# littlepure2333/GFlow

Measured on AMD Instinct MI355X. Metric: GFlow fit_video frames/sec (fwd+bwd+step) @60k Gaussians 480p, higher is better.
Workload: dtype f32

## Files before the change

gflow_amd/_lib.py:

```python
import ctypes
import os
import subprocess
import threading

import torch

_HERE = os.path.dirname(os.path.abspath(__file__))
_CSRC = os.path.join(_HERE, "csrc")
LIB_PATH = os.environ.get("GFLOW_HIP_LIB") or os.path.join(_HERE, "libgflow_hip.so")

_lock = threading.Lock()
_lib = None

c_void_p, c_int, c_float, c_size_t, c_int64 = ctypes.c_void_p, ctypes.c_int, ctypes.c_float, ctypes.c_size_t, ctypes.c_int64

MIN_VERSION = 312

_P = c_void_p
SIGNATURES = {
    "gfl_version": (c_int, []),
    "gfl_constants": (c_int, [_P]),
    "gfl_constants_n": (c_int, [_P, c_int]),
    "gfl_ewa_on_mfma": (c_int, []),
    "gfl_status_string": (ctypes.c_char_p, [c_int]),
# ... 26 lines not shown
    "gfl_step_increment": (c_int, [_P, _P]),
    "gfl_tile_sort_only": (c_int, [_P, c_int, c_int, _P, _P, _P, _P]),
    "gfl_tile_sort_ordered": (c_int, [_P, c_int, c_int, c_int, _P, _P, _P, _P]),
    "gfl_tile_sort_reserved": (c_int, [_P, _P, _P, _P, c_int, c_int, c_int, _P, _P, _P, _P]),
    "gfl_fit_workspace_bytes": (c_size_t, [c_int, c_int, c_int, c_int]),
    "gfl_fit_workspace_layout": (c_int, [c_int, c_int, c_int, c_int, _P, _P, _P, c_int]),
    "gfl_fit_forward": (c_int, [_P, _P, _P]),
    "gfl_fit_backward_step": (c_int, [_P, _P, _P]),
    "gfl_fit_iteration": (c_int, [_P, _P, _P]),
    "gfl_fit_iterations": (c_int, [_P, _P, c_int, c_int, _P]),
    "gfl_fit_reserved_supported": (c_int, [_P, _P]),
    "gfl_fit_snapshot_stage": (c_int, [_P, _P, _P]),
    "gfl_fit_snapshot_workspace_bytes": (c_size_t, [c_int, c_int, c_int]),
    "gfl_fit_snapshot": (c_int, [_P, _P, _P, _P, _P, c_size_t, _P]),
    "gfl_fit_iteration_snapshot": (c_int, [_P, _P, _P, _P, _P]),
    "gfl_render_fwd": (c_int, [_P, _P, _P]),
    "gfl_render_bwd": (c_int, [_P, _P, _P, _P, _P, _P, _P, _P]),
    "gfl_render_bwd_cam": (c_int, [_P, _P, _P, _P, _P, _P, _P, _P, _P]),
    "gfl_render_batch_workspace_bytes": (c_size_t, [c_int, c_int, c_int, c_int, c_int]),
    "gfl_render_batch": (c_int, [_P, c_int, _P, _P, c_int, c_int, c_int, c_int, c_int, _P, _P, _P, _P, _P, c_size_t, _P]),
    "gfl_fit_prepare_targets": (c_int, [_P, _P]),
    "gfl_fit_schedule_info": (c_int, [_P, _P, _P, _P, _P]),
    "gfl_fit_schedule_info_fwd": (c_int, [_P, _P, _P, _P, _P]),
    "gfl_selftest_reduce10": (c_int, [_P, _P, _P, _P]),
    "gfl_selftest_cov2d": (c_int, [_P, _P, c_int, _P, _P, _P]),
    "gfl_selftest_block_mask": (c_int, [_P, c_int, c_int, c_int, c_int, _P, _P, _P]),
    "gfl_concave_hull": (c_int, [_P, c_int, ctypes.c_double, ctypes.c_double, _P, c_int]),
    "gfl_scan_f64_workspace_bytes": (c_size_t, [c_int]),
    "gfl_scan_f64": (c_int, [_P, c_int, _P, _P, c_size_t, _P]),
    "gfl_track_anchor_workspace_bytes": (c_size_t, [c_int, c_int]),
# ... 142 lines not shown
```

gflow_amd/csrc/gfl_fit.hip:

```cpp
#include "gfl_fit_blend.hpp"

using namespace gfl;

extern "C" {

size_t gfl_loss_workspace_bytes(int W, int H);

static inline int fit_nblk(int N) { return (N + BIN_BLOCK - 1) / BIN_BLOCK; }

static bool ewa_on_mfma() {
    static const bool on = [] { const char* e = getenv("GFL_EWA_MFMA"); return e && e[0] == '1'; }();
    return on;
}

int gfl_ewa_on_mfma(void) { return ewa_on_mfma() ? 1 : 0; }

static int fwd_split_min() {
    static const int v = [] { const char* e = getenv("GFL_FWD_SPLIT_MIN"); return e ? atoi(e) : FWD_SPLIT_MIN; }();
    return v;
}

static bool reserved_enabled() {
    static const bool on = [] { const char* e = getenv("GFL_RESERVED"); return !(e && e[0] == '0'); }();
    return on;
}

static int device_cus() {
    static const int cus = [] {
        int dev = 0, n = 0;
        const bool ok = hipGetDevice(&dev) == hipSuccess &&
                        hipDeviceGetAttribute(&n, hipDeviceAttributeMultiprocessorCount, dev) == hipSuccess && n > 0;
        return ok ? n : 256;
    }();
    return cus;
// ... 155 lines not shown
static PreArgs pre_args(const gfl_fit_state* st, const gfl_fit_hyper* hp, const FitWs& w, int gx, int gy, int op_mode) {
    PreArgs a;
    a.intr = st->intr; a.pose = st->pose;
    a.N = st->N; a.W = st->W; a.H = st->H;
    a.nearest = hp->nearest; a.extent = hp->extent;
    a.gx = gx; a.gy = gy;
    a.rec = st->rec; a.wide_off = w.wide_off; a.hist_g = w.hist; a.extr_out = st->extr; a.overflow = st->overflow;
    a.pool_counter = w.pool_counter; a.pool_cap = st->K_cap;
    a.op_mode = op_mode;
    a.scale_rows_mode = (!op_mode && hp->lambda_scale != 0.f) ? (hp->freeze_all_splats ? 2 : 1) : 0;
    a.scale_cnt = w.scale_cnt;
    return a;
}

static int fit_forward_impl(const gfl_fit_state* st, const gfl_fit_hyper* hp, gfl_stream_t stream, int op_mode, int reserved = 0,
                            const float* snap_lut = nullptr, uint8_t* snap_u8 = nullptr) {
    int rc = fit_check(st, hp);
    if (rc) return rc;
    hipStream_t s = (hipStream_t)stream;
    const auto [gx, gy, T] = tile_grid(st->W, st->H);
    const FitWs w = carve(st);
    const int nblk = fit_nblk(st->N > 0 ? st->N : 1);
    if ((size_t)T * sizeof(int32_t) > 57 * 1024) return GFL_ERR_INVALID;
    const PreArgs pa = pre_args(st, hp, w, gx, gy, op_mode);
    if (reserved) {
        if (op_mode || !fit_reserved_ok(w, T)) return GFL_ERR_INVALID;
        {
            StageScope p(ST_PREPROCESS, s);
            BinArgs b;
            b.region = w.region; b.fill = w.fill; b.keys = w.keys; b.K_cap = st->K_cap;
            b.regions_valid = w.regions_valid; b.extent_next = w.extent_next; b.extent = w.extent;
// ... 27 lines not shown
                                           stream);
            else
                rc = gfl_tile_sort_only(st->tile_offsets, gx * gy, st->K_cap, w.keys, st->ids, st->tile_range, stream);
        }
        if (rc) return rc;
    }
    {
        StageScope p(ST_BLEND_FWD, s);
        const TileQueue q = {w.sched_fwd.list, w.sched_fwd.count, w.sched.counters, w.sched.nq, w.sched.cap_q};
        if (snap_u8) {
            rc = check(hipMemsetAsync(w.snap_mm, 0, 2 * sizeof(unsigned), s));
            if (rc) return rc;
            if (st->N > 0) launch_rec_depth_range(st->rec, st->N, w.snap_mm, s);
            launch_blend_fwd(st, hp->bg, gx, blend_grid(st, T, FWD_WG_PER_CU), st->render, st->final_T, st->n_contrib, q, w, 2,
                             w.snap_mm, snap_lut, fwd_split_min(), s, snap_u8);
            launch_center_blend(st, hp->bg, gx, T, nullptr, snap_u8 + (size_t)2 * st->W * st->H * 3, s);
        }
        const bool foot = st->foot_flags && !(hp->bg > 0.f) && st->N > 0;
        if (foot && !st->keep) return GFL_ERR_INVALID;
        const bool foot_inside = foot && !snap_u8;
        if (!snap_u8)
            launch_blend_fwd(st, hp->bg, gx, blend_grid(st, T, FWD_WG_PER_CU), st->render, st->final_T, st->n_contrib, q, w,
                             foot_inside ? 3 : 0, nullptr, nullptr, fwd_split_min(), s);
        if (st->foot_flags) {
            if (!st->keep) return GFL_ERR_INVALID;
            if (foot && !foot_inside) launch_footprint(st, gx, T, s);
        }
    }
    return check_launch();
}

// ... 15 lines not shown
}

int gfl_fit_snapshot(const gfl_fit_state* st, const gfl_fit_hyper* hp, const float* lut, uint8_t* out_u8, void* workspace,
                     size_t workspace_bytes, gfl_stream_t stream) {
    int rc = fit_check(st, hp);
    if (rc) return rc;
    if (!lut || !out_u8 || !workspace) return GFL_ERR_INVALID;
    if (workspace_bytes < gfl_fit_snapshot_workspace_bytes(st->N, st->W, st->H)) return GFL_ERR_WORKSPACE;
    hipStream_t s = (hipStream_t)stream;
    const auto [gx, gy, T] = tile_grid(st->W, st->H);
    const FitWs w = carve(st);
    const SnapWs sw = snap_ws(workspace, st->W, st->H);
    rc = check(hipMemsetAsync(workspace, 0, sw.head_bytes, s));
    if (rc) return rc;
    if (st->N > 0) launch_rec_depth_range(st->rec, st->N, sw.mm, s);
    launch_center_blend(st, hp->bg, gx, T, sw.img_c, nullptr, s);
    {
        const TileQueue q = {w.sched_fwd.list, w.sched_fwd.count, sw.pull, w.sched.nq, w.sched.cap_q};
        launch_blend_fwd(st, hp->bg, gx, blend_grid(st, T, FWD_WG_PER_CU), sw.img_dc, sw.fT, sw.nc, q, w, 1, sw.mm, lut, fwd_split_min(), s);
    }
    launch_snapshot_u8(st->render, sw.img_dc, sw.img_c, st->W * st->H, out_u8, s);
    return check_launch();
}

int gfl_fit_snapshot_stage(const gfl_fit_state* src, const gfl_fit_state* dst, gfl_stream_t stream) {
    if (!src || !dst || !src->workspace || !dst->workspace || !src->rec || !dst->rec || !src->ids || !dst->ids ||
        !src->tile_range || !dst->tile_range || !src->render || !dst->render || !src->tile_offsets)
        return GFL_ERR_INVALID;
    if (src->W != dst->W || src->H != dst->H || src->N != dst->N || dst->N > dst->cap || src->N > src->cap)
        return GFL_ERR_INVALID;
    if (!fit_ws_fits(src) || !fit_ws_fits(dst)) return GFL_ERR_WORKSPACE;
// ... 4 lines not shown
    StageCopy c;
    c.k_ptr = a.extent;
    c.ids_cap = (unsigned)min(src->K_cap, dst->K_cap);
    c.seg[0] = {(const uint32_t*)src->ids, (uint32_t*)dst->ids, 0u};
    c.seg[1] = {(const uint32_t*)src->rec, (uint32_t*)dst->rec, (unsigned)((size_t)src->N * REC)};
    c.seg[2] = {(const uint32_t*)src->tile_range, (uint32_t*)dst->tile_range, (unsigned)(2 * T)};
    c.seg[3] = {(const uint32_t*)src->render, (uint32_t*)dst->render, (unsigned)(3 * P)};
    c.seg[4] = {(const uint32_t*)a.sched_fwd.list, (uint32_t*)b.sched_fwd.list,
                (unsigned)((size_t)a.sched_fwd.nq * a.sched_fwd.cap_q)};
    c.seg[5] = {(const uint32_t*)a.sched_fwd.count, (uint32_t*)b.sched_fwd.count, (unsigned)a.sched_fwd.nq};
    c.seg[6] = {(const uint32_t*)a.sched.first_slot, (uint32_t*)b.sched.first_slot, (unsigned)T};
    launch_snapshot_stage(c, (hipStream_t)stream);
    return check_launch();
}

int gfl_render_fwd(const gfl_fit_state* st, const gfl_fit_hyper* hp, gfl_stream_t stream) {
    if (st && st->foot_flags) return GFL_ERR_INVALID;
    if (st && (st->flags & GFL_FIT_DETERMINISTIC)) {
        const int rc = fit_check(st, hp);
        if (rc) return rc;
        const int T = tile_grid(st->W, st->H).T;
        const FitWs w = carve(st);
        hipStream_t s = (hipStream_t)stream;
        if (check(hipMemsetAsync(w.sched.work, 0, 4 * (size_t)T * sizeof(int32_t), s)) ||
            check(hipMemsetAsync(w.sched_fwd.work, 0, 4 * (size_t)T * sizeof(int32_t), s)) ||
            check(hipMemsetAsync(w.sched_valid, 0, sizeof(int32_t), s)))
            return GFL_ERR_HIP;
    }
    return fit_forward_impl(st, hp, stream, 1);
}
// ... 103 lines not shown
    if (rc) return rc;
    const int T = tile_grid(st->W, st->H).T;
    const FitWs w = carve(st);
    const bool res_ok = fit_reserved_ok(w, T) && st->N > 0;
    if ((flags & GFL_ITER_RESERVED) && !res_ok) return GFL_ERR_INVALID;
    for (int j = 0; j < count; ++j) {
        const int reserved = res_ok && (j > 0 || (flags & GFL_ITER_RESERVED)) ? 1 : 0;
        rc = fit_forward_impl(st, hp, stream, 0, reserved);
        if (rc) return rc;
        rc = gfl_fit_backward_step(st, hp, stream);
        if (rc) return rc;
    }
    return GFL_OK;
}

int gfl_fit_iteration_snapshot(const gfl_fit_state* st, const gfl_fit_hyper* hp, const float* lut, uint8_t* out_u8,
                               gfl_stream_t stream) {
    if (!lut || !out_u8) return GFL_ERR_INVALID;
    int rc = fit_forward_impl(st, hp, stream, 0, 0, lut, out_u8);
    if (rc) return rc;
    return gfl_fit_backward_step(st, hp, stream);
}

int gfl_fit_reserved_supported(const gfl_fit_state* st, const gfl_fit_hyper* hp) {
    if (fit_check(st, hp) || st->N <= 0) return 0;
    const int T = tile_grid(st->W, st->H).T;
    return fit_reserved_ok(carve(st), T) ? 1 : 0;
}

int gfl_fit_prepare_targets(const gfl_fit_state* st, gfl_stream_t stream) {
    if (!st || st->W <= 0 || st->H <= 0 || !st->gt_rgb || !st->workspace) return GFL_ERR_INVALID;
    if (!fit_ws_fits(st)) return GFL_ERR_WORKSPACE;
    const FitWs w = carve(st);
    return gfl_loss_prepare_gt(st->gt_rgb, st->keep, st->W, st->H, w.gt_stats, stream);
}

// ... 41 lines not shown
```

gflow_amd/csrc/gfl_fit.hpp:

```cpp
#pragma once
#include "gfl_math.hpp"
#include "gfl_profile.hpp"
#include "gfl_sched.hpp"

#include <stdlib.h>

namespace gfl {

constexpr int BIN_BLOCK = 512;
#ifndef GFL_RBIN_BLOCK
#define GFL_RBIN_BLOCK 512
#endif
constexpr int RBIN_BLOCK = GFL_RBIN_BLOCK;
static_assert(RBIN_BLOCK == 256 || RBIN_BLOCK == 512, "two scale-row partials per 512 splats (PreArgs.scale_cnt)");
#ifndef GFL_WIDE_TILES
#define GFL_WIDE_TILES 16
#endif
constexpr int WIDE_TILES = GFL_WIDE_TILES;
constexpr int ROW = 16;
constexpr int REC = 12;
#ifndef GFL_PG_STRIDE
#define GFL_PG_STRIDE 12
#endif
constexpr int PG = GFL_PG_STRIDE;
// ... 145 lines not shown
    unsigned long long* keys;
    int K_cap;
    int32_t* regions_valid;
    const int32_t* extent_next;
    int32_t* extent;
    int32_t* pull_counters; int n_pull;
};

__host__ __device__ __forceinline__ int region_cap(int c) { return c + (c >> 2) + 32; }
struct ReserveOut { int4* region; int32_t* fill; int32_t* extent_next; int32_t* total; int K_cap; };

constexpr int BLEND_WG_PER_CU = 8;
constexpr int FWD_WG_PER_CU = 5;
constexpr int FWD_UNITS = 4;
constexpr int FWD_SPLIT_MIN = 448;
constexpr int FB = 256;
#ifndef GFL_FWD_LONG_BATCH
#define GFL_FWD_LONG_BATCH 256
#endif
constexpr int FBL = GFL_FWD_LONG_BATCH;
constexpr int FBB = 192;
constexpr int FBB_DET = 64;

struct WgVote {
    int32_t* cnt;
    int base0, base1, round;
};
__device__ __forceinline__ WgVote wg_vote_init(int32_t* lds2) {
    WgVote v;
    v.cnt = lds2; v.base0 = 0; v.base1 = 0; v.round = 0;
// ... 245 lines not shown
}

struct StageSeg { const uint32_t* src; uint32_t* dst; unsigned n; };
struct StageCopy { StageSeg seg[7]; const int32_t* k_ptr; unsigned ids_cap; };

void launch_preprocess_fwd(const float* params, const PreArgs& a, const uint8_t* row_flags, int nblk, bool mfma, hipStream_t s);
void launch_preprocess_bin(const float* params, const PreArgs& a, const uint8_t* row_flags, const BinArgs& b, int nblk, bool mfma,
                           hipStream_t s);
void launch_colscan(const FitWs& w, int nblk, int T, int32_t* overflow, hipStream_t s);
void launch_scatter(const gfl_fit_state* st, const FitWs& w, int nblk, int gx, int gy, bool ordered, hipStream_t s);
inline unsigned inv_of(int gx) { return (unsigned)((((unsigned long long)1 << 32) + (unsigned)gx - 1) / (unsigned)gx); }
void launch_blend_fwd(const gfl_fit_state* st, float bg, int gx, int grid, float* out, float* final_T, int32_t* n_contrib,
                      const TileQueue& q, const FitWs& w, int mode, const unsigned* cmap_mm, const float* cmap_lut, int split_min,
                      hipStream_t s, uint8_t* snap_u8 = nullptr);
void launch_footprint(const gfl_fit_state* st, int gx, int T, hipStream_t s);
void launch_center_blend(const gfl_fit_state* st, float bg, int gx, int T, float* out, uint8_t* out_u8, hipStream_t s);
void launch_rec_depth_range(const float* rec, int N, unsigned* mm, hipStream_t s);
void launch_snapshot_u8(const float* a, const float* b, const float* c, int P, uint8_t* out, hipStream_t s);
void launch_snapshot_stage(const StageCopy& c, hipStream_t s);
void launch_blend_bwd(const gfl_fit_state* st, float bg, int gx, int gy, int grid, int sums, const float* d_out, const TileQueue& q,
                      const FitWs& w, const LossTail& lt, hipStream_t s);
void launch_splat_bwd_adam(const gfl_fit_state* st, const FitWs& w, int gx, int gy, const RegCfg& rc, const AdamCfg& ac,
                           const NextSched& ns, int extra, size_t lds, hipStream_t s);
void launch_splat_bwd_op(const gfl_fit_state* st, const FitWs& w, int gx, int gy, const NextSched& ns, int extra, size_t lds,
                         const float* d_uv, const float* d_depth, float* d_params, float* d_extr, hipStream_t s);
void launch_splat_bwd_op_cam(const gfl_fit_state* st, const FitWs& w, int gx, int gy, const NextSched& ns, int extra, size_t lds,
                             const float* d_uv, const float* d_depth, float* d_params, float* d_extr, float* d_intr, hipStream_t s);
void launch_camera_adam(const gfl_fit_state* st, const FitWs& w, int rows, const float* p_ssim, int n_ssim, const float* p_grad,
                        int n_grad, const AdamCfg& ac_cam, const AdamCfg& ac_ab, int step_camera, hipStream_t s);
#ifdef GFL_TRACE
int read_phase_trace_bin(long long* out, int n_values);
// ... 8 lines not shown
```

gflow_amd/csrc/gfl_fit_snap.hip:

```cpp
#include "gfl_fit.hpp"

namespace gfl {

__global__ void __launch_bounds__(256) center_blend_kernel(const float* __restrict__ rec, const int32_t* __restrict__ ids,
                                                           const int32_t* __restrict__ tile_range, float bg, int W, int H, int gx,
                                                           float* __restrict__ out, uint8_t* __restrict__ out_u8) {
    __shared__ RecLDS recs[FB + 1];
    __shared__ unsigned char s_mask[FB];
    const int tile = blockIdx.x;
    const int tx = tile % gx, ty = tile / gx;
    const TilePixel px = tile_pixel(tx, ty, W, H);
    const float blob_cutoff = alpha_cutoff(1.f, 1.f);
    float T, a[3];
    plain_tile_blend<3>(ids, tile_range[2 * tile], tile_range[2 * tile + 1], tx, ty, pixf(px.px), pixf(px.py), px.inside, recs, s_mask,
                        [&](int g, float4& p0, float4& p1, float4& p2) {
                            const float4* r4 = reinterpret_cast<const float4*>(rec + (size_t)g * REC);
                            p0 = r4[0]; p1 = r4[1]; p2 = r4[2];
                            p0.z = 1.f; p0.w = 0.f; p1.x = 1.f; p1.y = 1.f;
                            p2.z = p2.z < 0.f ? p2.z : blob_cutoff;
                        }, T, a);
    if (px.inside) {
        const size_t pix = (size_t)px.py * W + px.px, plane = (size_t)H * W;
        const float o0 = fmaf(T, bg, a[0]), o1 = fmaf(T, bg, a[1]), o2 = fmaf(T, bg, a[2]);
        if (out_u8) {
            uint8_t* u = out_u8 + pix * 3;
            u[0] = img_u8(o0); u[1] = img_u8(o1); u[2] = img_u8(o2);
        } else {
            out[pix] = o0; out[plane + pix] = o1; out[2 * plane + pix] = o2;
        }
    }
}

__global__ void __launch_bounds__(256) rec_depth_range_kernel(const float* __restrict__ rec, int N, unsigned* __restrict__ mm) {
    unsigned lo = 0xffffffffu, hi = 0u;
    for (int i = blockIdx.x * blockDim.x + threadIdx.x; i < N; i += gridDim.x * blockDim.x) {
        const float x = rec[(size_t)i * REC + 9];
        const unsigned b = __float_as_uint(x);
// ... 29 lines not shown
__global__ void __launch_bounds__(256) snapshot_stage_kernel(StageCopy c) {
    const unsigned tid = blockIdx.x * blockDim.x + threadIdx.x, stride = gridDim.x * blockDim.x;
#pragma unroll
    for (int sgi = 0; sgi < 7; ++sgi) {
        const StageSeg sg = c.seg[sgi];
        unsigned n = sg.n;
        if (sgi == 0) n = min((unsigned)max(*c.k_ptr, 0), c.ids_cap);
        const unsigned n4 = n >> 2;
        const uint4* s4 = reinterpret_cast<const uint4*>(sg.src);
        uint4* d4 = reinterpret_cast<uint4*>(sg.dst);
        for (unsigned i = tid; i < n4; i += stride) d4[i] = s4[i];
        for (unsigned i = (n4 << 2) + tid; i < n; i += stride) sg.dst[i] = sg.src[i];
    }
}

void launch_center_blend(const gfl_fit_state* st, float bg, int gx, int T, float* out, uint8_t* out_u8, hipStream_t s) {
    center_blend_kernel<<<T, 256, 0, s>>>(st->rec, st->ids, st->tile_range, bg, st->W, st->H, gx, out, out_u8);
}

void launch_rec_depth_range(const float* rec, int N, unsigned* mm, hipStream_t s) {
    rec_depth_range_kernel<<<min((N + 255) / 256, 32), 256, 0, s>>>(rec, N, mm);
}

void launch_snapshot_u8(const float* a, const float* b, const float* c, int P, uint8_t* out, hipStream_t s) {
    snapshot_u8_kernel<<<(P + 255) / 256, 256, 0, s>>>(a, b, c, P, out);
}

void launch_snapshot_stage(const StageCopy& c, hipStream_t s) { snapshot_stage_kernel<<<1024, 256, 0, s>>>(c); }

}
```

gflow_amd/fused.py:

```python
import ctypes

import torch

from . import _lib as L
from .pinned import DeferredRead

ROW = 16
REC = 12
COLS = {"xyz": (0, 3), "scale": (3, 6), "rotate": (6, 10), "opacity": (10, 11), "rgb": (11, 14)}

_P = ctypes.c_void_p
_I = ctypes.c_int32


class FitState(ctypes.Structure):
    _fields_ = [("N", _I), ("cap", _I), ("W", _I), ("H", _I), ("K_cap", _I), ("gt_cached", _I),
                ("params", _P), ("adam_m", _P), ("adam_v", _P), ("rec", _P), ("d_rec", _P),
                ("flow_target", _P), ("flow_w", _P), ("still_target", _P), ("still_w", _P), ("row_flags", _P),
                ("pose", _P), ("pose_m", _P), ("pose_v", _P),
                ("depth_ab", _P), ("depth_ab_m", _P), ("depth_ab_v", _P),
                ("intr", _P), ("extr", _P), ("d_extr", _P), ("step", _P),
                ("gt_rgb", _P), ("gt_depth", _P), ("keep", _P), ("move_mask", _P), ("foot_flags", _P),
                ("render", _P), ("final_T", _P), ("n_contrib", _P),
                ("d_render", _P), ("err_px", _P), ("sums", _P),
# ... 15 lines not shown
def _declare(lib):
    if getattr(lib, "_fit_declared", False):
        return
    lib.gfl_fit_workspace_bytes.restype = ctypes.c_size_t
    lib.gfl_fit_workspace_bytes.argtypes = [ctypes.c_int] * 4
    for name in ("gfl_fit_forward", "gfl_fit_backward_step", "gfl_fit_iteration", "gfl_render_fwd"):
        fn = getattr(lib, name)
        fn.restype = ctypes.c_int
        fn.argtypes = [ctypes.POINTER(FitState), ctypes.POINTER(FitHyper), _P]
    lib.gfl_fit_iterations.restype = ctypes.c_int
    lib.gfl_fit_iterations.argtypes = [ctypes.POINTER(FitState), ctypes.POINTER(FitHyper), ctypes.c_int, ctypes.c_int, _P]
    lib.gfl_fit_snapshot.restype = ctypes.c_int
    lib.gfl_fit_snapshot.argtypes = [ctypes.POINTER(FitState), ctypes.POINTER(FitHyper), _P, _P, _P, ctypes.c_size_t, _P]
    lib.gfl_fit_iteration_snapshot.restype = ctypes.c_int
    lib.gfl_fit_iteration_snapshot.argtypes = [ctypes.POINTER(FitState), ctypes.POINTER(FitHyper), _P, _P, _P]
    lib.gfl_render_bwd.restype = ctypes.c_int
    lib.gfl_render_bwd.argtypes = [ctypes.POINTER(FitState), ctypes.POINTER(FitHyper), _P, _P, _P, _P, _P, _P]
    lib.gfl_render_bwd_cam.restype = ctypes.c_int
    lib.gfl_render_bwd_cam.argtypes = [ctypes.POINTER(FitState), ctypes.POINTER(FitHyper), _P, _P, _P, _P, _P, _P, _P]
    lib._fit_declared = True


PROFILE = {"mask": 0}

import gc as _gc
import threading as _threading

_GRAPH_LOCK = _threading.RLock()


# ... 274 lines not shown
        L.check(self.lib.gfl_fit_backward_step(ctypes.byref(self.state()), ctypes.byref(self.hp), L.stream()),
                "fit backward/step")
        self._reserved_N = self.N

    GFL_ITER_RESERVED = 8

    def _reserved_flag(self):
        if self._reserved_N != self.N or self.N <= 0:
            return 0
        key = (self.W, self.H, self.K_cap)
        if self._reserved_sup[0] != key:
            self._reserved_sup = (key, int(self.lib.gfl_fit_reserved_supported(ctypes.byref(self.state()),
                                                                                ctypes.byref(self.hp))))
        return self.GFL_ITER_RESERVED if self._reserved_sup[1] else 0

    def iteration(self, use_graph=False, count=1, snapshot=False, flags=0, reserved=None):
        if snapshot:
            from .color import lut
            assert count == 1
            if self._snap_out is None:
                self._snap_out = torch.empty(3, self.H, self.W, 3, dtype=torch.uint8, device=self.dev)
            snap_args = (L.ptr(lut("turbo", self.dev)), L.ptr(self._snap_out))
        reserved = 0 if (flags or reserved is False or snapshot) else self._reserved_flag()
        st, hp = self.state(), self.hp
        fn, args, what = ((self.lib.gfl_fit_iteration_snapshot, snap_args, "snapshot iteration") if snapshot else
                          (self.lib.gfl_fit_iterations, (count, int(flags) | reserved), "fit iterations"))
        launch = lambda: L.check(fn(ctypes.byref(st), ctypes.byref(hp), *args, L.stream()), what)
        if use_graph and not PROFILE["mask"] and self._launched and not flags:
            gkey = ("snap", count, reserved) if snapshot else (count, reserved)
            g = self.graphs.lookup(bytes(st) + bytes(hp), gkey)
            if g is None:
                g = self.graphs.capture(gkey, launch)
            g.replay()
        else:
            launch()
            self._launched = True
        self._reserved_N = self.N
        return self._snap_out if snapshot else None

    def snapshot(self, out=None):
        from .color import lut
        need = self.lib.gfl_fit_snapshot_workspace_bytes(self.N, self.W, self.H)
        if self._snap_ws is None or self._snap_ws.numel() < need:
            self._snap_ws = torch.empty(int(need * 1.5), dtype=torch.uint8, device=self.dev)
        if out is None:
            out = torch.empty(3, self.H, self.W, 3, dtype=torch.uint8, device=self.dev)
        L.check(self.lib.gfl_fit_snapshot(ctypes.byref(self.state()), ctypes.byref(self.hp), L.ptr(lut("turbo", self.dev)),
                                          L.ptr(out), L.ptr(self._snap_ws), self._snap_ws.numel(), L.stream()), "snapshot")
        return out

    _STATE_TENSORS = ("step", "pose", "pose_m", "pose_v", "depth_ab", "ab_m", "ab_v")

    def save_state(self):
        n = self.N
        out = {"N": n, "rows": [t[:n].clone() for t in (self.params, self.adam_m, self.adam_v)]}
        for k in self._STATE_TENSORS:
            out[k] = getattr(self, k).clone()
        return out

    def restore_state(self, saved):
        n = saved["N"]
        if n != self.N:
            raise RuntimeError("FitEngine.restore_state: the splat count has changed since save_state")
        self._reserved_N = -1
# ... 116 lines not shown
```

gflow_amd/stage.py:

```python
from types import SimpleNamespace

import torch

from . import geometry, losses
from . import render as render_mod
from .optim import LinearLR
from .pinned import PINNED, copy_stream


class StagePlan(SimpleNamespace):

    def snapshot(self, i):
        return bool(self.snapshot_interval) and i % self.snapshot_interval == 0

    def log(self, i):
        return bool(self.log_interval) and i % self.log_interval == 0

    def occ_densify(self, i):
        return bool(self.occlusion) and i == 0

    def err_densify(self, i):
        return bool(not self.camera_only and self.densify_interval and (i + 1) % self.densify_interval == 0
                    and (i + 1) // self.densify_interval <= self.densify_times)

# ... 267 lines not shown
                last()

    def account(self):
        k = self.eng.take_pending()
        if k is None:
            if self.unchecked:
                self.settle()
        elif k < 0:
            self.settle()
        else:
            for _ in range(k):
                self.eng.iteration(use_graph=False, reserved=False)

    def _launch(self, dst, n_rendered, looked_at):
        tr, eng = self.tr, self.eng
        if dst is not None and not tr.async_snapshots:
            imgs = eng.iteration(use_graph=tr.use_graph, snapshot=True, reserved=False)
            torch.bitwise_or(imgs, 0, out=dst)
        else:
            eng.iteration(use_graph=tr.use_graph, reserved=None if not looked_at else False)
            if dst is not None:
                tr._snapshot_async(dst, n_rendered)
                self.sink.snap_stream = tr._snap_stream

    def one_iteration(self):
        tr, eng, p, iteration = self.tr, self.eng, self.plan, self.iteration
        n_rendered = eng.N
        looked_at = not p.plain(iteration)
        if looked_at and tr.exact_snapshots:
            self.account()
        if self.tentative:
            tr.rasterisations_done += 1
        dst = None
        if p.snapshot(iteration):
            dst = self.sink.slot(len(self.frames))
        launch = lambda: self._launch(dst, n_rendered, looked_at)
        launch()
        if looked_at and tr.exact_snapshots == "blocking":
# ... 73 lines not shown
```

gflow_amd/trainer.py:

```python
import math
import os

import numpy as np
import torch
import torch.nn as nn
import torch.nn.functional as F

from . import _lib as L
from . import geometry, msplat
from . import render as render_mod
from .geometry import device_constant, pose_to_extr, rotmat_to_unitquat_xyzw
from .optim import Adam
from .pinned import PINNED
from .sampling import complex_texture_sampling
from .stage import FusedStage, OperatorStage, StagePlan


def run_to_end(g):
    try:
        while True:
            next(g)
    except StopIteration as e:
        return e.value


class SimpleGaussian:
    def __init__(self, gt_image, gt_depth=None, gt_flow=None, num_points=100000, background="black",
                 device=None, log_dir=None, seed=None, fused=True, deterministic=None):
        self.fused = bool(fused)
        self.deterministic = L.resolve_deterministic(deterministic)
        if self.deterministic and not self.fused and deterministic is not None:
            raise ValueError("SimpleGaussian(deterministic=True) needs fused=True: the operator path's alpha_blending "
                             "backward has no deterministic implementation")
        self.async_snapshots = True
        self.exact_snapshots = True
        self.cu_count = 0
        self.use_graph = True
        self.engine = None
        self.device = torch.device(device if device is not None else "cuda")
        if self.device.type != "cuda":
            raise RuntimeError("gflow_amd.trainer needs a HIP device (there is no CPU rasteriser)")
        self.gt_image = gt_image.to(self.device)
        self.gt_depth = gt_depth.to(self.device) if gt_depth is not None else None
        self.gt_flow = gt_flow.to(self.device) if gt_flow is not None else None
        self.num_points = num_points
        H, W, _ = gt_image.shape
        self.H, self.W = H, W
        self.bg = {"black": 0.0, "white": 1.0, "cyan": 0.33}.get(background, 0.0)
        fov = math.pi / 2.0
# ... 267 lines not shown
        return run_to_end(self.train_steps(*a, **kw))

    def train_steps(self, iterations=500, save_ckpt=False, ckpt_name="ckpt", snapshot_interval=10, render_parts=True,
                    lazy_images=False, chunk=None, move_seg=False, **kw):
        st = self.make_stepper(iterations=iterations, snapshot_interval=snapshot_interval, **kw)
        if chunk:
            st.yielding = True
            while st.iteration < iterations:
                st.run(min(int(chunk), iterations - st.iteration))
                yield
        else:
            st.run(iterations)
        self.train_log = st.log
        if self.fused and self.engine is not None:
            st.settle()
            if st.sink.snap_stream is not None:
                with torch.cuda.stream(st.sink.snap_stream):
                    self._snap_aux.watch_overflow()
        move_mask = kw.get("move_mask")
        if move_mask is not None:
            move_mask = move_mask.to(self.device).bool()

        self._project_appended(st)
        uv_d, depth_d = st.uv.clone(), st.depth.clone()
        if not st.camera_only:
            self._relabel_after_stage(uv_d, depth_d, move_mask, move_seg)
        parts, parts_block = (None, None, None, None), None
        if self.has_still and render_parts:
            parts, parts_block = self._render_parts(st.sink)
            self.rasterisations_done += 2
        self.last_render = st.last_render.clone()
        if save_ckpt:
            self.save_checkpoint(ckpt_name=ckpt_name)
# ... 49 lines not shown
        self.last_depth = depth_d
        self.last_xyz = self.get_attribute("xyz").detach()
        self.last_num = self.last_xyz.shape[0]

    def _render_parts(self, sink):
        if self.fused and self.engine is not None and self.engine.N == self.still_mask.shape[0]:
            block, pin = sink.copy_out(self._render_parts_fused())
            return pin, block
        with torch.no_grad():
            o = render_mod.render_multiple(self._input_group(sel=self.still_mask, detach=True), ["rgb", "center"])
            still_rgb, still_center = render_mod.render2img(o["rgb"]), render_mod.render2img(o["center"])
            o = render_mod.render_multiple(self._input_group(sel=~self.still_mask, detach=True), ["rgb", "center"])
            move_rgb, move_center = render_mod.render2img(o["rgb"]), render_mod.render2img(o["center"])
        return (still_rgb, still_center, move_rgb, move_center), None

    def _snapshot_async(self, out, n):
        import ctypes
        eng = self.engine
        cur = torch.cuda.current_stream()
        if not self._fits(self._snap_aux, n, eng.K_cap):
            if self._snap_aux is not None:
                self._snap_stream.synchronize()
            else:
                self._snap_stream = torch.cuda.Stream(device=self.device)
            self._snap_aux = self._new_engine(max(eng.cap, n), eng.K_cap)
            self._snap_done = None
        aux, side = self._snap_aux, self._snap_stream
        if self._snap_done is not None:
            cur.wait_event(self._snap_done)
        aux.set_count(n)
        aux.hp.bg, aux.hp.nearest, aux.hp.extent = eng.hp.bg, eng.hp.nearest, eng.hp.extent
        L.check(eng.lib.gfl_fit_snapshot_stage(ctypes.byref(eng.state()), ctypes.byref(aux.state()), L.stream()),
                "snapshot stage")
        ready = torch.cuda.Event()
        ready.record(cur)
        with torch.cuda.stream(side):
            side.wait_event(ready)
            aux.snapshot(out=out)
            self._snap_done = torch.cuda.Event()
            self._snap_done.record(side)

    @staticmethod
    def _fits(aux, n, K_cap=None):
        return aux is not None and aux.cap >= n and (K_cap is None or aux.K_cap >= K_cap)

    def _aux_engine(self):
        eng = self.engine
        if not self._fits(self._aux, eng.N):
            self._aux = self._new_engine(max(eng.cap, eng.N))
        aux = self._aux
        aux.set_count(eng.N)
        aux.pose.copy_(eng.pose)
        aux.intr.copy_(eng.intr)
        aux.hp.bg = self.bg
        return aux
# ... 187 lines not shown
```

include/gflow_hip.h:

```cpp
#ifndef GFLOW_HIP_H
#define GFLOW_HIP_H

#include <stddef.h>
#include <stdint.h>

#ifdef __cplusplus
extern "C" {
#endif

typedef void* gfl_stream_t;

typedef enum gfl_status {
    GFL_OK = 0,
    GFL_ERR_INVALID = -1,
    GFL_ERR_WORKSPACE = -2,
    GFL_ERR_HIP = -3
} gfl_status;

#define GFL_TILE 16
#ifndef GFL_NEAREST
#define GFL_NEAREST 0.2f
#endif
#ifndef GFL_EXTENT
#define GFL_EXTENT 1.3f
// ... 159 lines not shown
int gfl_render_fwd(const gfl_fit_state* st, const gfl_fit_hyper* hp, gfl_stream_t stream);
int gfl_render_bwd(const gfl_fit_state* st, const gfl_fit_hyper* hp, const float* d_render, const float* d_uv,
                   const float* d_depth, float* d_params, float* d_extr, gfl_stream_t stream);
int gfl_render_bwd_cam(const gfl_fit_state* st, const gfl_fit_hyper* hp, const float* d_render, const float* d_uv,
                       const float* d_depth, float* d_params, float* d_extr, float* d_intr, gfl_stream_t stream);
size_t gfl_render_batch_workspace_bytes(int J, int rows_total, int K_cap, int W, int H);
int gfl_render_batch(const float* params, int R, const int32_t* job_rows, const float* job_cam, int J, int rows_total, int W,
                     int H, int K_cap, float* out_f32, uint8_t* out_u8, float* out_rec, int32_t* overflow, void* workspace,
                     size_t workspace_bytes, gfl_stream_t stream);
size_t gfl_fit_snapshot_workspace_bytes(int N, int W, int H);
int gfl_fit_snapshot(const gfl_fit_state* st, const gfl_fit_hyper* hp, const float* lut, uint8_t* out_u8, void* workspace,
                     size_t workspace_bytes, gfl_stream_t stream);
int gfl_fit_iteration_snapshot(const gfl_fit_state* st, const gfl_fit_hyper* hp, const float* lut, uint8_t* out_u8,
                               gfl_stream_t stream);
int gfl_fit_snapshot_stage(const gfl_fit_state* src, const gfl_fit_state* dst, gfl_stream_t stream);
int gfl_fit_prepare_targets(const gfl_fit_state* st, gfl_stream_t stream);
int gfl_fit_schedule_info(const gfl_fit_state* st, int* n_queues, int* queue_capacity, const int32_t** d_lists,
                          const int32_t** d_counts);
int gfl_fit_schedule_info_fwd(const gfl_fit_state* st, int* n_queues, int* queue_capacity, const int32_t** d_lists,
                              const int32_t** d_counts);
int gfl_tile_sort_only(const int32_t* tile_offsets, int T, int K_cap, void* keys, int32_t* ids,
                       int32_t* tile_range, gfl_stream_t stream);
#define GFL_SORT_MAX_SPLIT 64
#define GFL_SORT_ORDER_TRAILER (GFL_SORT_MAX_SPLIT + 4)
int gfl_tile_sort_ordered(const int32_t* order, int W, int H, int K_cap, void* keys, int32_t* ids, int32_t* tile_range,
                          gfl_stream_t stream);
int gfl_tile_sort_reserved(const int32_t* order, const int32_t* fill, int32_t* tile_counts, int32_t* void_words, int W, int H,
                           int K_cap, void* keys, int32_t* ids, int32_t* tile_range, gfl_stream_t stream);

int gfl_selftest_reduce10(const float* in, float* out_scatter, float* out_dpp, gfl_stream_t stream);
// ... 62 lines not shown
```

Baseline: 10.36.

## Move center-blend snapshot to side stream and split heavy tiles into quarters

On snapshot iterations the main stream now renders only the RGB and depth snapshot images inside the fused forward pass. It stages ids, rec and tile_range into a shadow state, and the center-blob render plus the image copy run on a side stream so they overlap with the backward and step. The center blend kernel also gains a split path: tiles with more than split_min splats are handled by four blocks, each covering an 8x8 quarter with wave-level masks, which balances long tiles. This adds launch overhead (4*T blocks, most exiting early) and a staging copy, and adds a cross-stream dependency.

```diff
diff --git a/gflow_amd/_lib.py b/gflow_amd/_lib.py
--- a/gflow_amd/_lib.py
+++ b/gflow_amd/_lib.py
@@ -64,6 +64,10 @@
     "gfl_fit_snapshot_workspace_bytes": (c_size_t, [c_int, c_int, c_int]),
     "gfl_fit_snapshot": (c_int, [_P, _P, _P, _P, _P, c_size_t, _P]),
     "gfl_fit_iteration_snapshot": (c_int, [_P, _P, _P, _P, _P]),
+    "gfl_fit_iteration_snapshot_flags": (c_int, [_P, _P, _P, _P, c_int, _P]),
+    "gfl_fit_center": (c_int, [_P, _P, _P, _P]),
+    "gfl_fit_center_stage": (c_int, [_P, _P, _P]),
+    "gfl_fit_center_split_min": (c_int, [c_int]),
     "gfl_render_fwd": (c_int, [_P, _P, _P]),
     "gfl_render_bwd": (c_int, [_P, _P, _P, _P, _P, _P, _P, _P]),
     "gfl_render_bwd_cam": (c_int, [_P, _P, _P, _P, _P, _P, _P, _P, _P]),
diff --git a/gflow_amd/csrc/gfl_fit.hip b/gflow_amd/csrc/gfl_fit.hip
--- a/gflow_amd/csrc/gfl_fit.hip
+++ b/gflow_amd/csrc/gfl_fit.hip
@@ -1,3 +1,5 @@
+#include <atomic>
+
 #include "gfl_fit_blend.hpp"
 
 using namespace gfl;
@@ -18,6 +20,16 @@
 static int fwd_split_min() {
     static const int v = [] { const char* e = getenv("GFL_FWD_SPLIT_MIN"); return e ? atoi(e) : FWD_SPLIT_MIN; }();
     return v;
+}
+
+static std::atomic<int>& center_split_min_ref() {
+    static std::atomic<int> v{[] { const char* e = getenv("GFL_CENTER_SPLIT_MIN"); return e ? atoi(e) : CENTER_SPLIT_MIN; }()};
+    return v;
+}
+static int center_split_min() { return center_split_min_ref().load(std::memory_order_relaxed); }
+
+int gfl_fit_center_split_min(int value) {
+    return value < 0 ? center_split_min() : center_split_min_ref().exchange(value, std::memory_order_relaxed);
 }
 
 static bool reserved_enabled() {
@@ -203,7 +215,7 @@
 }
 
 static int fit_forward_impl(const gfl_fit_state* st, const gfl_fit_hyper* hp, gfl_stream_t stream, int op_mode, int reserved = 0,
-                            const float* snap_lut = nullptr, uint8_t* snap_u8 = nullptr) {
+                            const float* snap_lut = nullptr, uint8_t* snap_u8 = nullptr, bool snap_center = true) {
     int rc = fit_check(st, hp);
     if (rc) return rc;
     hipStream_t s = (hipStream_t)stream;
@@ -261,7 +273,8 @@
             if (st->N > 0) launch_rec_depth_range(st->rec, st->N, w.snap_mm, s);
             launch_blend_fwd(st, hp->bg, gx, blend_grid(st, T, FWD_WG_PER_CU), st->render, st->final_T, st->n_contrib, q, w, 2,
                              w.snap_mm, snap_lut, fwd_split_min(), s, snap_u8);
-            launch_center_blend(st, hp->bg, gx, T, nullptr, snap_u8 + (size_t)2 * st->W * st->H * 3, s);
+            if (snap_center)
+                launch_center_blend(st, hp->bg, gx, T, center_split_min(), nullptr, snap_u8 + (size_t)2 * st->W * st->H * 3, s);
         }
         const bool foot = st->foot_flags && !(hp->bg > 0.f) && st->N > 0;
         if (foot && !st->keep) return GFL_ERR_INVALID;
@@ -307,7 +320,7 @@
     rc = check(hipMemsetAsync(workspace, 0, sw.head_bytes, s));
     if (rc) return rc;
     if (st->N > 0) launch_rec_depth_range(st->rec, st->N, sw.mm, s);
-    launch_center_blend(st, hp->bg, gx, T, sw.img_c, nullptr, s);
+    launch_center_blend(st, hp->bg, gx, T, center_split_min(), sw.img_c, nullptr, s);
     {
         const TileQueue q = {w.sched_fwd.list, w.sched_fwd.count, sw.pull, w.sched.nq, w.sched.cap_q};
         launch_blend_fwd(st, hp->bg, gx, blend_grid(st, T, FWD_WG_PER_CU), sw.img_dc, sw.fT, sw.nc, q, w, 1, sw.mm, lut, fwd_split_min(), s);
@@ -342,6 +355,33 @@
     return check_launch();
 }
 
+int gfl_fit_center_stage(const gfl_fit_state* src, const gfl_fit_state* dst, gfl_stream_t stream) {
+    if (!src || !dst || !src->workspace || !src->rec || !dst->rec || !src->ids || !dst->ids || !src->tile_range ||
+        !dst->tile_range)
+        return GFL_ERR_INVALID;
+    if (src->W != dst->W || src->H != dst->H || src->N != dst->N || src->N < 0 || dst->N > dst->cap || src->N > src->cap ||
+        src->K_cap < 0 || dst->K_cap < 0)
+        return GFL_ERR_INVALID;
+    if (!fit_ws_fits(src)) return GFL_ERR_WORKSPACE;
+    const int T = tile_grid(src->W, src->H).T;
+    const FitWs a = carve(src);
+    StageCopy c = {};
+    c.k_ptr = a.extent;
+    c.ids_cap = (unsigned)min(src->K_cap, dst->K_cap);
+    c.seg[0] = {(const uint32_t*)src->ids, (uint32_t*)dst->ids, 0u};
+    c.seg[1] = {(const uint32_t*)src->rec, (uint32_t*)dst->rec, (unsigned)((size_t)src->N * REC)};
+    c.seg[2] = {(const uint32_t*)src->tile_range, (uint32_t*)dst->tile_range, (unsigned)(2 * T)};
+    launch_snapshot_stage(c, (hipStream_t)stream);
+    return check_launch();
+}
+
+int gfl_fit_center(const gfl_fit_state* st, const gfl_fit_hyper* hp, uint8_t* out_u8, gfl_stream_t stream) {
+    if (!st || !hp || !out_u8 || !st->rec || !st->ids || !st->tile_range || st->W <= 0 || st->H <= 0 || st->N < 0) return GFL_ERR_INVALID;
+    const auto [gx, gy, T] = tile_grid(st->W, st->H);
+    launch_center_blend(st, hp->bg, gx, T, center_split_min(), nullptr, out_u8, (hipStream_t)stream);
+    return check_launch();
+}
+
 int gfl_render_fwd(const gfl_fit_state* st, const gfl_fit_hyper* hp, gfl_stream_t stream) {
     if (st && st->foot_flags) return GFL_ERR_INVALID;
     if (st && (st->flags & GFL_FIT_DETERMINISTIC)) {
@@ -475,12 +515,17 @@
     return GFL_OK;
 }
 
+int gfl_fit_iteration_snapshot_flags(const gfl_fit_state* st, const gfl_fit_hyper* hp, const float* lut, uint8_t* out_u8, int flags,
+                                     gfl_stream_t stream) {
+    if (!lut || !out_u8 || (flags & ~GFL_SNAP_NO_CENTER)) return GFL_ERR_INVALID;
+    int rc = fit_forward_impl(st, hp, stream, 0, 0, lut, out_u8, !(flags & GFL_SNAP_NO_CENTER));
+    if (rc) return rc;
+    return gfl_fit_backward_step(st, hp, stream);
+}
+
 int gfl_fit_iteration_snapshot(const gfl_fit_state* st, const gfl_fit_hyper* hp, const float* lut, uint8_t* out_u8,
                                gfl_stream_t stream) {
-    if (!lut || !out_u8) return GFL_ERR_INVALID;
-    int rc = fit_forward_impl(st, hp, stream, 0, 0, lut, out_u8);
-    if (rc) return rc;
-    return gfl_fit_backward_step(st, hp, stream);
+    return gfl_fit_iteration_snapshot_flags(st, hp, lut, out_u8, 0, stream);
 }
 
 int gfl_fit_reserved_supported(const gfl_fit_state* st, const gfl_fit_hyper* hp) {
diff --git a/gflow_amd/csrc/gfl_fit.hpp b/gflow_amd/csrc/gfl_fit.hpp
--- a/gflow_amd/csrc/gfl_fit.hpp
+++ b/gflow_amd/csrc/gfl_fit.hpp
@@ -183,6 +183,7 @@
 constexpr int FWD_WG_PER_CU = 5;
 constexpr int FWD_UNITS = 4;
 constexpr int FWD_SPLIT_MIN = 448;
+constexpr int CENTER_SPLIT_MIN = 256;
 constexpr int FB = 256;
 #ifndef GFL_FWD_LONG_BATCH
 #define GFL_FWD_LONG_BATCH 256
@@ -458,7 +459,7 @@
                       const TileQueue& q, const FitWs& w, int mode, const unsigned* cmap_mm, const float* cmap_lut, int split_min,
                       hipStream_t s, uint8_t* snap_u8 = nullptr);
 void launch_footprint(const gfl_fit_state* st, int gx, int T, hipStream_t s);
-void launch_center_blend(const gfl_fit_state* st, float bg, int gx, int T, float* out, uint8_t* out_u8, hipStream_t s);
+void launch_center_blend(const gfl_fit_state* st, float bg, int gx, int T, int split_min, float* out, uint8_t* out_u8, hipStream_t s);
 void launch_rec_depth_range(const float* rec, int N, unsigned* mm, hipStream_t s);
 void launch_snapshot_u8(const float* a, const float* b, const float* c, int P, uint8_t* out, hipStream_t s);
 void launch_snapshot_stage(const StageCopy& c, hipStream_t s);
diff --git a/gflow_amd/csrc/gfl_fit_snap.hip b/gflow_amd/csrc/gfl_fit_snap.hip
--- a/gflow_amd/csrc/gfl_fit_snap.hip
+++ b/gflow_amd/csrc/gfl_fit_snap.hip
@@ -2,25 +2,111 @@
 
 namespace gfl {
 
+
+__device__ __forceinline__ void blob_record(float4& p0, float4& p1, float4& p2, float blob_cutoff) {
+    p0.z = 1.f; p0.w = 0.f; p1.x = 1.f; p1.y = 1.f;
+    p2.z = p2.z < 0.f ? p2.z : blob_cutoff;
+}
+
+template <typename Stage>
+__device__ __forceinline__ void center_quarter_blend(const int32_t* __restrict__ ids, int start, int end, int bx0, int by0, float fx,
+                                                     float fy, bool inside, RecLDS* recs, unsigned char* s_mask, Stage&& stage,
+                                                     float& T, float (&acc)[3]) {
+    const int tid = threadIdx.x, wave = tid >> 6, lane = tid & 63, row = lane >> 4;
+    if (tid == 0) {
+        const float4 z = make_float4(0.f, 0.f, 0.f, 0.f);
+        recs[FB].p0 = z; recs[FB].p1 = z; recs[FB].p2 = z;
+    }
+    T = 1.f;
+    float Tw = inside ? 1.f : 0.f;
+#pragma unroll
+    for (int n = 0; n < 3; ++n) acc[n] = 0.f;
+    for (int base = start; base < end; base += FB) {
+        if (__syncthreads_and(Tw == 0.f)) break;
+        const int idx = base + tid;
+        unsigned char m = 0;
+        if (idx < end) {
+            float4 p0, p1, p2;
+            stage(ids[idx], p0, p1, p2);
+            recs[tid].p0 = p0; recs[tid].p1 = p1; recs[tid].p2 = p2;
+            m = (unsigned char)block_mask(p0, p1, p2.z, bx0, by0, 4);
+        }
+        s_mask[tid] = m;
+        __syncthreads();
+        const int cnt = min(FB, end - base);
+        for (int c0 = 0; c0 < cnt && !__all(Tw == 0.f); c0 += 64) {
+            const int slot = c0 + lane;
+            unsigned long long bits = __ballot(slot < cnt && ((s_mask[slot] >> wave) & 1));
+            while (bits) {
+                int j[4];
+#pragma unroll
+                for (int k = 0; k < 4; ++k) {
+                    j[k] = bits ? c0 + (int)__builtin_ctzll(bits) : FB;
+                    bits &= bits - 1;
+                }
+                const int js = row == 0 ? j[0] : (row == 1 ? j[1] : (row == 2 ? j[2] : j[3]));
+                float al, G;
+                const bool val = splat_alpha2(recs[js].p0, recs[js].p1, fx, fy, al, G);
+                const float a_mine = val ? al : 0.f;
+                float lo = a_mine, hi = a_mine;
+                permlane32_swap(lo, hi);
+                float av[4] = {lo, lo, hi, hi};
+                permlane16_swap(av[0], av[1]);
+                permlane16_swap(av[2], av[3]);
+                float feat[4][3];
+#pragma unroll
+                for (int k = 0; k < 4; ++k) { feat[k][0] = recs[j[k]].p1.z; feat[k][1] = recs[j[k]].p1.w; feat[k][2] = recs[j[k]].p2.x; }
+#pragma unroll
+                for (int k = 0; k < 4; ++k) {
+                    const float a = av[k];
+                    const float test_T = Tw * (1.f - a);
+                    const bool stop = test_T < GFL_T_MIN;
+                    const float w = stop ? 0.f : a * Tw;
+#pragma unroll
+                    for (int n = 0; n < 3; ++n) acc[n] = fmaf(feat[k][n], w, acc[n]);
+                    T = stop ? T : test_T;
+                    Tw = stop ? 0.f : test_T;
+                }
+                if (__all(Tw == 0.f)) break;
+            }
+        }
+    }
+}
+
 __global__ void __launch_bounds__(256) center_blend_kernel(const float* __restrict__ rec, const int32_t* __restrict__ ids,
                                                            const int32_t* __restrict__ tile_range, float bg, int W, int H, int gx,
-                                                           float* __restrict__ out, uint8_t* __restrict__ out_u8) {
+                                                           int n_tiles, int split_min, float* __restrict__ out,
+                                                           uint8_t* __restrict__ out_u8) {
     __shared__ RecLDS recs[FB + 1];
     __shared__ unsigned char s_mask[FB];
-    const int tile = blockIdx.x;
+    const int part = (int)blockIdx.x / n_tiles, tile = (int)blockIdx.x - part * n_tiles;
+    const int start = tile_range[2 * tile], end = tile_range[2 * tile + 1];
+    const bool split = end - start > split_min;
+    if (part > 0 && !split) return;
     const int tx = tile % gx, ty = tile / gx;
-    const TilePixel px = tile_pixel(tx, ty, W, H);
     const float blob_cutoff = alpha_cutoff(1.f, 1.f);
+    auto stage = [&](int g, float4& p0, float4& p1, float4& p2) {
+        const float4* r4 = reinterpret_cast<const float4*>(rec + (size_t)g * REC);
+        p0 = r4[0]; p1 = r4[1]; p2 = r4[2];
+        blob_record(p0, p1, p2, blob_cutoff);
+    };
+    int px, py;
+    bool inside, writer = true;
     float T, a[3];
-    plain_tile_blend<3>(ids, tile_range[2 * tile], tile_range[2 * tile + 1], tx, ty, pixf(px.px), pixf(px.py), px.inside, recs, s_mask,
-                        [&](int g, float4& p0, float4& p1, float4& p2) {
-                            const float4* r4 = reinterpret_cast<const float4*>(rec + (size_t)g * REC);
-                            p0 = r4[0]; p1 = r4[1]; p2 = r4[2];
-                            p0.z = 1.f; p0.w = 0.f; p1.x = 1.f; p1.y = 1.f;
-                            p2.z = p2.z < 0.f ? p2.z : blob_cutoff;
-                        }, T, a);
-    if (px.inside) {
-        const size_t pix = (size_t)px.py * W + px.px, plane = (size_t)H * W;
+    if (split) {
+        const int wave = threadIdx.x >> 6, lane = threadIdx.x & 63;
+        const int bx0 = tx * GFL_TILE + (part & 1) * 8, by0 = ty * GFL_TILE + (part >> 1) * 8;
+        px = bx0 + (wave & 1) * 4 + (lane & 3); py = by0 + (wave >> 1) * 4 + ((lane >> 2) & 3);
+        inside = px < W && py < H;
+        writer = lane < 16;
+        center_quarter_blend(ids, start, end, bx0, by0, pixf(px), pixf(py), inside, recs, s_mask, stage, T, a);
+    } else {
+        const TilePixel tp = tile_pixel(tx, ty, W, H);
+        px = tp.px; py = tp.py; inside = tp.inside;
+        plain_tile_blend<3>(ids, start, end, tx, ty, pixf(px), pixf(py), inside, recs, s_mask, stage, T, a);
+    }
+    if (inside && writer) {
+        const size_t pix = (size_t)py * W + px, plane = (size_t)H * W;
         const float o0 = fmaf(T, bg, a[0]), o1 = fmaf(T, bg, a[1]), o2 = fmaf(T, bg, a[2]);
         if (out_u8) {
             uint8_t* u = out_u8 + pix * 3;
@@ -80,8 +166,9 @@
     }
 }
 
-void launch_center_blend(const gfl_fit_state* st, float bg, int gx, int T, float* out, uint8_t* out_u8, hipStream_t s) {
-    center_blend_kernel<<<T, 256, 0, s>>>(st->rec, st->ids, st->tile_range, bg, st->W, st->H, gx, out, out_u8);
+void launch_center_blend(const gfl_fit_state* st, float bg, int gx, int T, int split_min, float* out, uint8_t* out_u8, hipStream_t s) {
+    if (T <= 0) return;
+    center_blend_kernel<<<4 * T, 256, 0, s>>>(st->rec, st->ids, st->tile_range, bg, st->W, st->H, gx, T, split_min, out, out_u8);
 }
 
 void launch_rec_depth_range(const float* rec, int N, unsigned* mm, hipStream_t s) {
diff --git a/gflow_amd/fused.py b/gflow_amd/fused.py
--- a/gflow_amd/fused.py
+++ b/gflow_amd/fused.py
@@ -53,6 +53,12 @@
     lib.gfl_fit_snapshot.argtypes = [ctypes.POINTER(FitState), ctypes.POINTER(FitHyper), _P, _P, _P, ctypes.c_size_t, _P]
     lib.gfl_fit_iteration_snapshot.restype = ctypes.c_int
     lib.gfl_fit_iteration_snapshot.argtypes = [ctypes.POINTER(FitState), ctypes.POINTER(FitHyper), _P, _P, _P]
+    lib.gfl_fit_iteration_snapshot_flags.restype = ctypes.c_int
+    lib.gfl_fit_iteration_snapshot_flags.argtypes = [ctypes.POINTER(FitState), ctypes.POINTER(FitHyper), _P, _P, ctypes.c_int, _P]
+    lib.gfl_fit_center.restype = ctypes.c_int
+    lib.gfl_fit_center.argtypes = [ctypes.POINTER(FitState), ctypes.POINTER(FitHyper), _P, _P]
+    lib.gfl_fit_center_stage.restype = ctypes.c_int
+    lib.gfl_fit_center_stage.argtypes = [ctypes.POINTER(FitState), ctypes.POINTER(FitState), _P]
     lib.gfl_render_bwd.restype = ctypes.c_int
     lib.gfl_render_bwd.argtypes = [ctypes.POINTER(FitState), ctypes.POINTER(FitHyper), _P, _P, _P, _P, _P, _P]
     lib.gfl_render_bwd_cam.restype = ctypes.c_int
@@ -357,20 +363,22 @@
                                                                                 ctypes.byref(self.hp))))
         return self.GFL_ITER_RESERVED if self._reserved_sup[1] else 0
 
-    def iteration(self, use_graph=False, count=1, snapshot=False, flags=0, reserved=None):
+    GFL_SNAP_NO_CENTER = 1
+
+    def iteration(self, use_graph=False, count=1, snapshot=False, flags=0, reserved=None, center=True):
         if snapshot:
             from .color import lut
             assert count == 1
             if self._snap_out is None:
                 self._snap_out = torch.empty(3, self.H, self.W, 3, dtype=torch.uint8, device=self.dev)
-            snap_args = (L.ptr(lut("turbo", self.dev)), L.ptr(self._snap_out))
+            snap_args = (L.ptr(lut("turbo", self.dev)), L.ptr(self._snap_out), 0 if center else self.GFL_SNAP_NO_CENTER)
         reserved = 0 if (flags or reserved is False or snapshot) else self._reserved_flag()
         st, hp = self.state(), self.hp
-        fn, args, what = ((self.lib.gfl_fit_iteration_snapshot, snap_args, "snapshot iteration") if snapshot else
+        fn, args, what = ((self.lib.gfl_fit_iteration_snapshot_flags, snap_args, "snapshot iteration") if snapshot else
                           (self.lib.gfl_fit_iterations, (count, int(flags) | reserved), "fit iterations"))
         launch = lambda: L.check(fn(ctypes.byref(st), ctypes.byref(hp), *args, L.stream()), what)
         if use_graph and not PROFILE["mask"] and self._launched and not flags:
-            gkey = ("snap", count, reserved) if snapshot else (count, reserved)
+            gkey = ("snap", count, reserved, bool(center)) if snapshot else (count, reserved)
             g = self.graphs.lookup(bytes(st) + bytes(hp), gkey)
             if g is None:
                 g = self.graphs.capture(gkey, launch)
@@ -391,6 +399,13 @@
         L.check(self.lib.gfl_fit_snapshot(ctypes.byref(self.state()), ctypes.byref(self.hp), L.ptr(lut("turbo", self.dev)),
                                           L.ptr(out), L.ptr(self._snap_ws), self._snap_ws.numel(), L.stream()), "snapshot")
         return out
+
+    def center(self, out):
+        L.check(self.lib.gfl_fit_center(ctypes.byref(self.state()), ctypes.byref(self.hp), L.ptr(out), L.stream()), "center")
+        return out
+
+    def stage_center(self, dst):
+        L.check(self.lib.gfl_fit_center_stage(ctypes.byref(self.state()), ctypes.byref(dst.state()), L.stream()), "center stage")
 
     _STATE_TENSORS = ("step", "pose", "pose_m", "pose_v", "depth_ab", "ab_m", "ab_v")
 
diff --git a/gflow_amd/stage.py b/gflow_amd/stage.py
--- a/gflow_amd/stage.py
+++ b/gflow_amd/stage.py
@@ -305,14 +305,18 @@
 
     def _launch(self, dst, n_rendered, looked_at):
         tr, eng = self.tr, self.eng
-        if dst is not None and not tr.async_snapshots:
-            imgs = eng.iteration(use_graph=tr.use_graph, snapshot=True, reserved=False)
+        if dst is None:
+            eng.iteration(use_graph=tr.use_graph, reserved=None if not looked_at else False)
+            return
+        side = tr.async_snapshots and tr.center_placement == "side"
+        if side:
+            tr._center_async_wait()
+        imgs = eng.iteration(use_graph=tr.use_graph, snapshot=True, reserved=False, center=not side)
+        if side:
+            tr._center_async(dst, imgs, n_rendered)
+            self.sink.snap_stream = tr._snap_stream
+        else:
             torch.bitwise_or(imgs, 0, out=dst)
-        else:
-            eng.iteration(use_graph=tr.use_graph, reserved=None if not looked_at else False)
-            if dst is not None:
-                tr._snapshot_async(dst, n_rendered)
-                self.sink.snap_stream = tr._snap_stream
 
     def one_iteration(self):
         tr, eng, p, iteration = self.tr, self.eng, self.plan, self.iteration
diff --git a/gflow_amd/trainer.py b/gflow_amd/trainer.py
--- a/gflow_amd/trainer.py
+++ b/gflow_amd/trainer.py
@@ -33,6 +33,7 @@
             raise ValueError("SimpleGaussian(deterministic=True) needs fused=True: the operator path's alpha_blending "
                              "backward has no deterministic implementation")
         self.async_snapshots = True
+        self.center_placement = os.environ.get("GFLOW_CENTER_PLACEMENT", "side")
         self.exact_snapshots = True
         self.cu_count = 0
         self.use_graph = True
@@ -330,9 +331,6 @@
         self.train_log = st.log
         if self.fused and self.engine is not None:
             st.settle()
-            if st.sink.snap_stream is not None:
-                with torch.cuda.stream(st.sink.snap_stream):
-                    self._snap_aux.watch_overflow()
         move_mask = kw.get("move_mask")
         if move_mask is not None:
             move_mask = move_mask.to(self.device).bool()
@@ -412,8 +410,24 @@
             move_rgb, move_center = render_mod.render2img(o["rgb"]), render_mod.render2img(o["center"])
         return (still_rgb, still_center, move_rgb, move_center), None
 
-    def _snapshot_async(self, out, n):
-        import ctypes
+    def _center_async_wait(self):
+        if self._snap_done is not None:
+            torch.cuda.current_stream().wait_event(self._snap_done)
+
+    def _center_async(self, out, imgs, n):
+        eng, cur = self.engine, torch.cuda.current_stream()
+        aux, side = self._snap_shadow(n)
+        eng.stage_center(aux)
+        ready = torch.cuda.Event()
+        ready.record(cur)
+        with torch.cuda.stream(side):
+            side.wait_event(ready)
+            aux.center(out[2])
+            torch.bitwise_or(imgs[:2], 0, out=out[:2])
+            self._snap_done = torch.cuda.Event()
+            self._snap_done.record(side)
+
+    def _snap_shadow(self, n):
         eng = self.engine
         cur = torch.cuda.current_stream()
         if not self._fits(self._snap_aux, n, eng.K_cap):
@@ -428,15 +442,7 @@
             cur.wait_event(self._snap_done)
         aux.set_count(n)
         aux.hp.bg, aux.hp.nearest, aux.hp.extent = eng.hp.bg, eng.hp.nearest, eng.hp.extent
-        L.check(eng.lib.gfl_fit_snapshot_stage(ctypes.byref(eng.state()), ctypes.byref(aux.state()), L.stream()),
-                "snapshot stage")
-        ready = torch.cuda.Event()
-        ready.record(cur)
-        with torch.cuda.stream(side):
-            side.wait_event(ready)
-            aux.snapshot(out=out)
-            self._snap_done = torch.cuda.Event()
-            self._snap_done.record(side)
+        return aux, side
 
     @staticmethod
     def _fits(aux, n, K_cap=None):
diff --git a/include/gflow_hip.h b/include/gflow_hip.h
--- a/include/gflow_hip.h
+++ b/include/gflow_hip.h
@@ -197,6 +197,12 @@
 int gfl_fit_iteration_snapshot(const gfl_fit_state* st, const gfl_fit_hyper* hp, const float* lut, uint8_t* out_u8,
                                gfl_stream_t stream);
 int gfl_fit_snapshot_stage(const gfl_fit_state* src, const gfl_fit_state* dst, gfl_stream_t stream);
+#define GFL_SNAP_NO_CENTER 1
+int gfl_fit_iteration_snapshot_flags(const gfl_fit_state* st, const gfl_fit_hyper* hp, const float* lut, uint8_t* out_u8, int flags,
+                                     gfl_stream_t stream);
+int gfl_fit_center(const gfl_fit_state* st, const gfl_fit_hyper* hp, uint8_t* out_u8, gfl_stream_t stream);
+int gfl_fit_center_stage(const gfl_fit_state* src, const gfl_fit_state* dst, gfl_stream_t stream);
+int gfl_fit_center_split_min(int value);
 int gfl_fit_prepare_targets(const gfl_fit_state* st, gfl_stream_t stream);
 int gfl_fit_schedule_info(const gfl_fit_state* st, int* n_queues, int* queue_capacity, const int32_t** d_lists,
                           const int32_t** d_counts);
```

After: 10.12. 2.3% lower.
